# nextpyp/pyp

Measured on AMD Instinct MI355X. Metric: particles/sec projection-matching, 256^2 box, higher is better.
Workload: dtype f32

## Files before the change

pyp_amd/csrc/host_ctx.h:

```cpp
#pragma once

namespace {

thread_local std::string g_err;
int fail(int code, const std::string &msg) { g_err = "ERROR: " + msg; return code; }

#define HIPCHK(call)                                                                          \
    do {                                                                                      \
        hipError_t e_ = (call);                                                               \
        if (e_ != hipSuccess) {                                                               \
            g_err = std::string("ERROR: HIP: ") + hipGetErrorString(e_) + " at " #call;        \
            return -5;                                                                        \
        }                                                                                     \
    } while (0)
#define HIPCHKP(call)                                                                         \
    do {                                                                                      \
        hipError_t e_ = (call);                                                               \
        if (e_ != hipSuccess) {                                                               \
            g_err = std::string("ERROR: HIP: ") + hipGetErrorString(e_) + " at " #call;        \
            return nullptr;                                                                   \
        }                                                                                     \
    } while (0)

struct Ctx {
// ... 112 lines not shown
        if (n <= cap) return 0;
        if (p) (void)hipFree(p);
        p = nullptr; cap = 0;
        HIPCHK(hipMalloc(&p, n * sizeof(T)));
        cap = n;
        return 0;
    }
    void release() { if (p) (void)hipFree(p); p = nullptr; cap = 0; }
};

template <typename T>
struct DevTmp {
    T *p = nullptr;
    DevTmp() = default;
    DevTmp(const DevTmp &) = delete;
    DevTmp &operator=(const DevTmp &) = delete;
    ~DevTmp() { if (p) (void)hipFree(p); }
    hipError_t alloc(size_t n) { return hipMalloc(&p, n * sizeof(T)); }
};


}

struct ppm_ref {
    hipStream_t stream = nullptr, copy = nullptr;
    int N = 0, B = 0, CX = 0, CY = 0, NBX = 0, NBY = 0, pad = 1; unsigned LB = 0;
    float2 *cube = nullptr;
    DevBuf<double> rows_in, rows_out, dir_theta, dir_phi;
    DevBuf<float> images, wring, cw, C2, nP, nI, cc, mats, ddef;
    DevBuf<float2> c_Il, c_band; DevBuf<float> c_cw, c_img, c_wring; DevBuf<double> c_rows, c_N, c_p, c_tl, c_delta, c_s0, c_g0, c_out;
    DevBuf<int> c_eval, c_rp, c_rt, c_slot, c_uoff, c_active; DevBuf<LState> c_states; DevBuf<double> c_mean, c_tmean, c_acc, c_dtrial, c_fpm, c_delta_t;
    DevBuf<float2> s_f, s_g, s_F; DevBuf<float> s_vols;
    struct { bool valid = false; float key[5] = { 0, 0, 0, 0, 0 }; int S = 0; std::vector<int> shell_off; DevBuf<uint32_t> samples, pos; DevBuf<float> bandw; DevBuf<float2> Fw; bool fw_valid = false; float wkey[4] = { 0, 0, 0, 0 }; } s_plan;
    DevBuf<float2> band, Il, Wp, bank, twN;
    DevBuf<float2> spill;
    DevBuf<float4> rowtw;
    DevBuf<int> sh;
    DevBuf<uint32_t> samples;
    DevBuf<Hit> hits, hits_t;
    DevBuf<int> tile_c;
    DevBuf<Hit> hits_s; DevBuf<int> sec_k;
    DevBuf<LState> states, states2;
    DevBuf<float4> bank4; DevBuf<float> part, gtw;
    std::string grid_key, bank_key, bank4_key; int gtw_ns = 0, gtw_rsx = -1;
    long last_counts[4] = { 0, 0, 0, 0 };
    int last_sections = 0;
    std::string note;
};

struct ppm_accum {
    hipStream_t stream = nullptr, copy = nullptr;
    int N = 0; float pixel = 1.f;
    float *acc = nullptr; bool external = false;
    std::vector<double> symops; int nsym = 1;
    float *d_sym = nullptr;
    unsigned long long *d_counts = nullptr;
    unsigned *d_max = nullptr;
    long counts[2] = { 0, 0 };
    DevBuf<double> rows; DevBuf<float> images, dose; DevBuf<float2> band, spill; DevBuf<PartIns> pp; DevBuf<CullEnt> cull; DevBuf<BrickItem> items;
    DevBuf<float2> s_f, s_g; DevBuf<float> s_vols;
    std::vector<float> brick_load; float load_r = -1.f; int n_items = 0, items_cap = -1;
};

static CubeView cube_view(const ppm_ref *ref) {
    CubeView cv;
// ... 4 lines not shown
static bool local_tables_wanted(int tabR) {
    return !(getenv("PPM_LOCAL_TABLES") && atoi(getenv("PPM_LOCAL_TABLES")) == 0) && cube_tab_bytes(tabR) <= 16 * 1024;
}
static bool tables_fit_lds(size_t ring_bytes, int tabR) { return ring_bytes + cube_tab_bytes(tabR) + 2048 <= (size_t)64 * 1024; }

struct ChunkStager {
    const float *src; float *buf; bool on_device; int n_img, chunk; size_t nn;
    int prime() const {
        if (on_device) return 0;
        HIPCHK(hipMemcpyAsync(buf, src, (size_t)std::min(chunk, n_img) * nn * sizeof(float), hipMemcpyHostToDevice, cur_copy()));
        HIPCHK(hipStreamSynchronize(cur_copy()));
        return 0;
    }
    const float *chunk_ptr(int c0, int ci) const { return on_device ? src + (size_t)c0 * nn : buf + (size_t)(ci & 1) * chunk * nn; }
    int prefetch_next(int c0, int ci) const {
        if (on_device || c0 + chunk >= n_img) return 0;
        const int n_next = std::min(chunk, n_img - (c0 + chunk));
        HIPCHK(hipMemcpyAsync(buf + (size_t)((ci + 1) & 1) * chunk * nn, src + (size_t)(c0 + chunk) * nn, (size_t)n_next * nn * sizeof(float), hipMemcpyHostToDevice, cur_copy()));
        return 0;
    }
    int sync() const {
        HIPCHK(hipStreamSynchronize(cur_stream()));
        HIPCHK(hipStreamSynchronize(cur_copy()));
        return 0;
    }
};

static __global__ void k_noop() {}

extern "C" {

const char *ppm_last_error(void) { return g_err.c_str(); }
const char *ppm_version(void) { return "pypmatch 0.1 (gfx950)"; }
const char *ppm_build_id(void) { return "pypmatch " __DATE__ " " __TIME__; }
int ppm_device_mem_info(size_t *free_bytes, size_t *total_bytes) {
    if (!g.inited) return fail(-1, "ppm_init has not been called");
    (void)hipSetDevice(g.device);
    size_t f = 0, t = 0;
    HIPCHK(hipMemGetInfo(&f, &t));
    if (free_bytes) *free_bytes = f;
    if (total_bytes) *total_bytes = t;
    return 0;
}

int ppm_init(int device) {
    static std::mutex init_mu;
// ... 149 lines not shown
```

pyp_amd/csrc/host_refine.h:

```cpp
#pragma once

static int launch_prep(DevBuf<float2> &spill , const float *d_images, const double *d_rows, int n_img, const Geom &gm, double Rm_px, float fall_px,
                       int normalize, int invert, int do_mask, int whiten, float2 *band, float *wring,
                       const uint32_t *samples, int S_pad, float2 *Il, float *cw, float2 *Wp, float *C2, float *nI,
                       unsigned *band_max = nullptr ,
                       const float *focus_px = nullptr ) {
    if (int rc = ensure_plan(gm.N)) return rc;
    PrepP P;
    P.images = d_images; P.rows = d_rows; P.plan = g.plans[gm.N].plan;
    P.N = gm.N; P.B = gm.B; P.W = gm.W; P.H = gm.H;
    P.r_hi2 = (float)(gm.r_hi * gm.r_hi); P.Rm = (float)Rm_px; P.wfall = fall_px; P.a = (float)gm.a;
    P.Rm2_bg = (float)std::min(std::floor(Rm_px * Rm_px), 16777216.0);
    P.normalize = normalize; P.invert = invert; P.do_mask = do_mask; P.whiten = whiten;
    for (int k = 0; k < 4; k++) P.focus[k] = focus_px ? focus_px[k] : 0.f;
    P.band_max = band_max;
    P.band = band; P.wring = wring; P.samples = samples; P.S_pad = S_pad; P.Il = Il; P.cw = cw;
    P.Wp = Wp; P.C2 = C2; P.nI = nI; P.Bs = gm.Bs; P.Hs = gm.Hs;
    P.r_s2 = (float)(gm.r_s * gm.r_s); P.r_lo2 = (float)(gm.r_lo * gm.r_lo);
    const PrepPlan pl = prep_plan(gm.N, gm.B, gm.W);
    if (pl.err) return fail(-12, pl.err);
    P.L = pl.L; P.nc = pl.nc; P.nchunks = pl.nchunks; P.TS = pl.TS; P.WS = pl.WS;
    P.spill = nullptr;
    if (!pl.scratch_free) {
        if (int rc = spill.ensure((size_t)n_img * gm.N * gm.W)) return rc;
// ... 121 lines not shown
    DP.rlo2 = (float)(gm.r_lo * gm.r_lo); DP.rmax2 = (float)(gm.r_hi * gm.r_hi); DP.ring_signed = (float)std::min(gm.ring_signed, 1e30); DP.a = (float)gm.a;
    DP.rows = rows; DP.states = states; DP.ddef = ddef; DP.nt = nt; DP.step = step; DP.all_scores = all_scores; DP.rcls2 = rcls2;
    DP.tchunk = std::max(1, std::min(2 * nt + 1, (int)(60000 / (16 * (size_t)nrings))));
    ProfScope ps(PPM_K_LOCAL);
    hipLaunchKernelGGL(k_defocus, dim3(n), dim3(256), ring_lds_bytes(4, DP.tchunk, nrings), cur_stream(), DP);
}

namespace {
struct RefineRun {
    ppm_ref *ref = nullptr; const ppm_refine_cfg *cfg = nullptr;
    Geom gm; SampleList sl; CubeView cv;
    int S_pad = 0, nrings = 0, CH = 0;
    int K = 0, Tb = 0, Tc = 0;
    double Rm_px = 0; float fall_px = 0;
    bool focus_on = false, sep_search = false; float focus_px[4] = { 0, 0, 0, 0 };
    GfftPlan gpl; bool use_fft = false;
    int Rtx = 0, Rty = 0, Rwin = 0, HsP = 0, nslices = 0; std::vector<int> cxs, cys;
    std::vector<GridSection> secs; std::vector<int> kpre; int sec_dirs = 0;
    LocalP LP; bool local_tab = false;
    double bf = 3.0; bool any_ang = false, any_sh = false;
    int ndef = 0;
    int per_iter = 0; bool cls_on = false;
    double sample_evals = 0;

    int ntiles() const { return (int)(cxs.size() * cys.size()); }
    int nsec() const { return (int)secs.size(); }
    size_t bank_slice() const { return (size_t)HsP * 64; }
    size_t bank4_slice() const { return use_fft ? (size_t)gpl.L * gpl.L : 0; }
    size_t HS() const { return (size_t)gm.Hs * 64; }
    int prefix_of(double rband) const { int rg = (int)std::ceil(rband); if (rg > gm.B + 1) rg = gm.B + 1; return sl.ring_off[rg]; }
};
constexpr int kTileR = 6;
constexpr int kFinalThreads = 256;
}

static void refine_notes(ppm_ref *ref, const ppm_refine_cfg *cfg, const Geom &gm) {
    ref->note.clear();
    if (gm.r_s_asked > gm.r_s) {
        char b[256];
        std::snprintf(b, sizeof(b), "NOTE: global search band lowered from %.1f to %.1f Fourier pixels (%.2f A instead of %.2f A): the grid-search "
                      "kernel covers 64 pixels; the top hits are refined up to the high-resolution limit as asked", gm.r_s_asked, gm.r_s,
                      gm.N * gm.a / gm.r_s, gm.N * gm.a / gm.r_s_asked);
        ref->note = b;
    }
    if (cfg->global_search && gm.range_capped) {
        char b[320];
        std::snprintf(b, sizeof(b), "%sNOTE: shift window of the grid search: +-%.0f x +-%.0f pixels (%d x %d search-grid steps of %.1f pixels, the most the "
                      "search grid of %d points holds; asked: %.0f pixels); the refinement of the hits is not limited to it", ref->note.empty() ? "" : "\n",
                      gm.RSx * gm.step, gm.RSy * gm.step, gm.RSx, gm.RSy, gm.step, gm.Ns, gm.range_asked_px);
        ref->note += b;
    }
}

static size_t workspace_budget() { return g.total_mem / 4; }
static size_t bank_budget() {
    size_t b = g.total_mem / 4;
// ... 49 lines not shown
    HIPCHK(hipMemcpyAsync(ref->samples.p, r.sl.packed.data(), r.S_pad * sizeof(uint32_t), hipMemcpyHostToDevice, cur_stream()));

    r.use_fft = false;
    if (cfg->global_search && gfft_plan(gm, r.gpl)) {
        const char *gp = getenv("PPM_GLOBAL_PATH");
        const bool force_fft = gp && !strcmp(gp, "fft"), force_tiles = gp && !strcmp(gp, "tiles");
        r.use_fft = force_fft || (!force_tiles && std::max(gm.RSx, gm.RSy) > kTileR);
    }
    r.Rtx = std::min(gm.RSx, kTileR); r.Rty = std::min(gm.RSy, kTileR);
    auto tile_centres = [](int RS, int Rt) {
        const int T = (2 * RS + 1 + 2 * Rt) / (2 * Rt + 1);
        std::vector<int> c(T, 0);
        for (int i = 0; i < T && T > 1; i++) c[i] = -RS + Rt + (int)(((long)i * 2 * (RS - Rt)) / (T - 1));
        return c;
    };
    r.cxs = tile_centres(gm.RSx, r.Rtx); r.cys = tile_centres(gm.RSy, r.Rty);
    r.Rwin = std::max(r.Rtx, r.Rty);
    r.HsP = ((2 * (gm.Bs + 1) + 2 * global_unroll(r.Rwin) - 1) / (2 * global_unroll(r.Rwin))) * (2 * global_unroll(r.Rwin));
    r.nslices = gm.n_dir * gm.npsi_store;
    if (cfg->global_search) if (int rc = plan_grid_sections(r)) return rc;
    const size_t NN = (size_t)gm.N * gm.N, HW = (size_t)gm.H * gm.W;
    size_t per = NN * 4 + HW * 8 + (size_t)r.S_pad * 12 + 2 * PPM_NCOL * 8 + (gm.B + 2) * 4;
    if (cfg->global_search) per += r.HS() * 12 + (size_t)r.nslices * 4 + (size_t)gm.n_orient * 8 + (size_t)r.K * (sizeof(Hit) + sizeof(LState)) + sizeof(LState);
    size_t fit = ((size_t)4 << 30) / per;
    if (fit < 64) {
        const size_t ws = workspace_budget(), per_all = per + (r.use_fft ? (size_t)gm.n_orient * 8 : 0);
        fit = std::min<size_t>(64, ws / per_all);
        if (fit < 1) {
            char b[320];
            std::snprintf(b, sizeof(b), "angular step of %.3g degrees: the grid search keeps %.1f GB of tables per particle for its %d orientations, "
                          "the workspace holds %.1f GB; use a coarser angular step", gm.dstep, per_all / 1073741824.0, gm.n_orient, ws / 1073741824.0);
            return fail(-22, b);
        }
    }
    int CH = (int)std::min<size_t>((size_t)n_img, fit);
    CH = std::min(CH, 8192);
    if (CH >= 2048) CH &= ~1023;
    if (const char *e = std::getenv("PPM_CHUNK")) { int v = std::atoi(e); if (v > 0) CH = std::min(CH, v); }
    r.CH = CH;
    return 0;
}

static int ensure_chunk_buffers(RefineRun &r, bool images_on_device) {
    ppm_ref *ref = r.ref; const Geom &gm = r.gm; const int CH = r.CH;
    const size_t NN = (size_t)gm.N * gm.N, HW = (size_t)gm.H * gm.W;
    if (int rc = ref->rows_in.ensure((size_t)CH * PPM_NCOL)) return rc;
    if (int rc = ref->rows_out.ensure((size_t)CH * PPM_NCOL)) return rc;
    if (!images_on_device) if (int rc = ref->images.ensure((size_t)2 * CH * NN)) return rc;
    if (int rc = ref->band.ensure((size_t)CH * HW)) return rc;
    if (int rc = ref->wring.ensure((size_t)CH * (gm.B + 2))) return rc;
    if (int rc = ref->Il.ensure((size_t)CH * r.S_pad)) return rc;
    if (int rc = ref->cw.ensure((size_t)CH * r.S_pad)) return rc;
    if (int rc = ref->states2.ensure(CH)) return rc;
    return 0;
}

static int ensure_bank(RefineRun &r, const GridSection &sec) {
    ppm_ref *ref = r.ref; const Geom &gm = r.gm;
    const std::string key = ref->grid_key + "/d" + std::to_string(sec.d0) + "+" + std::to_string(sec.nd);
    if (ref->bank_key == key) return 0;
    const int nsl = sec.nd * gm.npsi_store;
    BankP BP; BP.cv = r.cv; BP.mats = ref->mats.p + (size_t)sec.d0 * gm.npsi_store * 6; BP.bank = ref->bank.p; BP.nslices = nsl; BP.Bs = gm.Bs; BP.Hs = r.HsP;
    BP.r_s2 = (float)(gm.r_s * gm.r_s);
    {
        ProfScope ps(PPM_K_BANK);
        size_t tot = (size_t)nsl * r.bank_slice();
        hipLaunchKernelGGL(k_bank, dim3((unsigned)((tot + 255) / 256)), dim3(256), 0, cur_stream(), BP);
    }
    HIPCHK(hipGetLastError());
    ref->bank_key = key;
    return 0;
}

static int ensure_bank4(RefineRun &r, const GridSection &sec) {
    ppm_ref *ref = r.ref; const Geom &gm = r.gm; const int L = r.gpl.L;
    const std::string key = ref->grid_key + "/d" + std::to_string(sec.d0) + "+" + std::to_string(sec.nd) + "/L" + std::to_string(L);
    if (ref->bank4_key == key) return 0;
    const int nsl = sec.nd * gm.npsi_store;
    Bank4P BP; BP.cv = r.cv; BP.mats = ref->mats.p + (size_t)sec.d0 * gm.npsi_store * 6; BP.bank4 = ref->bank4.p; BP.nslices = nsl; BP.Bs = gm.Bs; BP.L = L; BP.r_s2 = (float)(gm.r_s * gm.r_s);
    ProfScope ps(PPM_K_BANK);
    const size_t tot = (size_t)nsl * r.bank4_slice();
    hipLaunchKernelGGL(k_bank4, dim3((unsigned)((tot + 255) / 256)), dim3(256), 0, cur_stream(), BP);
    HIPCHK(hipGetLastError());
    ref->bank4_key = key;
    return 0;
}

static int ensure_search_tables(RefineRun &r) {
    ppm_ref *ref = r.ref; const Geom &gm = r.gm; const int CH = r.CH, K = r.K, nslices = r.nslices, HsP = r.HsP;
    const size_t HS = r.HS(), HSP = (size_t)HsP * 64;
    if (int rc = ref->Wp.ensure((size_t)CH * HS)) return rc;
    if (int rc = ref->C2.ensure((size_t)CH * HS)) return rc;
    if (int rc = ref->nP.ensure((size_t)CH * nslices)) return rc;
    if (int rc = ref->nI.ensure(CH)) return rc;
    if (int rc = ref->cc.ensure((size_t)CH * gm.n_orient)) return rc;
    if (int rc = ref->sh.ensure((size_t)CH * gm.n_orient)) return rc;
    if (int rc = ref->hits.ensure((size_t)CH * K)) return rc;
    if (int rc = ref->states.ensure((size_t)CH * K)) return rc;
    {
        const size_t cap = ref->bank.cap;
        if (int rc = ref->bank.ensure((size_t)r.sec_dirs * gm.npsi_store * HSP)) return rc;
        if (ref->bank.cap != cap) ref->bank_key.clear();
    }
    if (r.nsec() > 1) {
        if (int rc = ref->hits_s.ensure((size_t)CH * r.kpre.back())) return rc;
        if (int rc = ref->sec_k.ensure(r.kpre.size())) return rc;
        HIPCHK(hipMemcpyAsync(ref->sec_k.p, r.kpre.data(), r.kpre.size() * sizeof(int), hipMemcpyHostToDevice, cur_stream()));
    }
    char key[160];
    std::snprintf(key, sizeof(key), "%d/%.6f/%.6f/%d/%d/%d/%.3f/%.3f", gm.N, gm.r_s, gm.dstep, gm.Ns, gm.npsi_store, HsP, gm.phi_max, gm.theta_max);
    if (ref->grid_key == key) return 0;
    ref->bank_key.clear(); ref->bank4_key.clear();
    std::vector<float> mats((size_t)nslices * 6);
    std::vector<double> dth(gm.n_dir), dph(gm.n_dir);
    for (int d = 0; d < gm.n_dir; d++) {
        grid_direction(gm, d, dth[d], dph[d]);
        for (int k = 0; k < gm.npsi_store; k++) {
            double M[9]; euler_matrix(k * gm.dpsi, dth[d], dph[d], M);
            float *m = &mats[((size_t)d * gm.npsi_store + k) * 6];
            m[0] = (float)M[0]; m[1] = (float)M[1]; m[2] = (float)M[3]; m[3] = (float)M[4]; m[4] = (float)M[6]; m[5] = (float)M[7];
        }
// ... 41 lines not shown
                for (int j = 1; j <= 3; j++) put(&tw[(size_t)fr::bfly_entry(L, M, k) * 8 + (j - 1) * 2], 2.0 * kPi * j * k / M);
        for (int t = 0; t < L; t++) put(&tw[(size_t)nb * 8 + (size_t)t * 2], 2.0 * kPi * t / gm.Ns);
        for (int pp = 0; pp < L; pp++)
            for (int h = 0; h < 2; h++) {
                const int j = 2 * fr::freq_at(L, pp) + h, sx = j < L ? j : j - gm.Ns;
                tw[(size_t)fr::tw_table_floats(L) + 2 * pp + h] = std::abs(sx) <= gm.RSx ? 0.f : -3.0e38f;
            }
        if (int rc = ref->gtw.ensure(tw.size())) return rc;
        HIPCHK(hipMemcpyAsync(ref->gtw.p, tw.data(), tw.size() * sizeof(float), hipMemcpyHostToDevice, cur_stream()));
        HIPCHK(hipStreamSynchronize(cur_stream()));
        ref->gtw_ns = gm.Ns; ref->gtw_rsx = gm.RSx;
    }
    return 0;
}

static int local_setup(RefineRun &r) {
    ppm_ref *ref = r.ref; const ppm_refine_cfg *cfg = r.cfg; const Geom &gm = r.gm; LocalP &LP = r.LP;
    r.bf = cfg->band_factor == 0 ? 3.0 : cfg->band_factor;
    r.any_ang = cfg->refine_psi || cfg->refine_theta || cfg->refine_phi; r.any_sh = cfg->refine_x || cfg->refine_y;
    r.sample_evals = 0;
    r.ndef = 0;
    if (cfg->refine_defocus && cfg->defocus_step > 0 && cfg->defocus_range >= cfg->defocus_step)
        r.ndef = std::min((int)std::floor(cfg->defocus_range / cfg->defocus_step + 1e-6), PPM_MAX_DEFOCUS_STEPS);
    LP.cv = r.cv; LP.samples = ref->samples.p; LP.Il = ref->Il.p; LP.cw = ref->cw.p; LP.S_pad = r.S_pad; LP.nrings = r.nrings; LP.N = gm.N;
    LP.tabR = cube_tab_radius(gm.B, r.cv.scale);
    r.local_tab = local_tables_wanted(LP.tabR);
    LP.rlo2 = (float)(gm.r_lo * gm.r_lo); LP.ring_signed = (float)std::min(gm.ring_signed, 1e30);
    LP.en[0] = cfg->refine_psi; LP.en[1] = cfg->refine_theta; LP.en[2] = cfg->refine_phi; LP.en[3] = cfg->refine_x; LP.en[4] = cfg->refine_y;
    LP.use_priors = 0;
    for (int i = 0; i < 5; i++) { LP.pmean[i] = 0; LP.pw[i] = 0; }
    if (cfg->use_priors) {
        const double ns = kPi * (gm.r_hi * gm.r_hi - gm.r_lo * gm.r_lo);
        for (int i = 0; i < 5; i++) {
            double var = cfg->prior_var[i], mean = cfg->prior_mean[i];
            if (i >= 3) { mean /= gm.a; var /= gm.a * gm.a; }
            LP.pmean[i] = mean;
            if (LP.en[i] && var > 0 && ns > 0) { LP.pw[i] = 1.0 / (2.0 * var * ns); LP.use_priors = 1; }
        }
    }
    const int nfree = (cfg->refine_psi != 0) + (cfg->refine_theta != 0) + (cfg->refine_phi != 0) + (cfg->refine_x != 0) + (cfg->refine_y != 0);
    r.per_iter = nfree ? 2 * nfree + 2 : 0;
    if (r.Tb + r.Tc > kMaxIters) return fail(-22, "too many compass iterations requested");
    LP.rmax2_final = (float)(gm.r_hi * gm.r_hi); LP.S_final = r.S_pad;
    r.cls_on = gm.r_cls < gm.r_hi;
    LP.rmax2_class = (float)(gm.r_cls * gm.r_cls); LP.S_class = (r.cls_on && r.ndef == 0) ? r.prefix_of(gm.r_cls) : 0;
    return 0;
}
// ... 43 lines not shown
    } else if (ntiles == 1) {
        if (int rc = launch_global(GP, nb, gm.half != 0, r.Rwin)) return rc;
    } else {
        if (int rc = ref->hits_t.ensure((size_t)ntiles * nb * K)) return rc;
        if (int rc = ref->tile_c.ensure((size_t)2 * ntiles)) return rc;
        std::vector<int> tc(2 * ntiles);
        for (int ty = 0, t = 0; ty < (int)r.cys.size(); ty++) for (int tx = 0; tx < (int)r.cxs.size(); tx++, t++) { tc[t] = r.cxs[tx]; tc[ntiles + t] = r.cys[ty]; }
        HIPCHK(hipMemcpyAsync(ref->tile_c.p, tc.data(), tc.size() * sizeof(int), hipMemcpyHostToDevice, cur_stream()));
        int px = 0, py = 0;
        const size_t tot = (size_t)nb * r.HS();
        for (int t = 0; t < ntiles; t++) {
            const int dcx = tc[t] - px, dcy = tc[ntiles + t] - py;
            if (dcx || dcy) hipLaunchKernelGGL(k_wp_ramp, dim3((unsigned)((tot + 255) / 256)), dim3(256), 0, cur_stream(), ref->Wp.p, tot, gm.Bs, gm.Ns, dcx, dcy, ref->twN.p);
            px = tc[t]; py = tc[ntiles + t];
            GP.hits = ref->hits_t.p + (size_t)t * nb * K;
            if (int rc = launch_global(GP, nb, gm.half != 0, r.Rwin)) return rc;
        }
        hipLaunchKernelGGL(k_merge_hits, dim3((nb + 127) / 128), dim3(128), 0, cur_stream(), ref->hits_t.p, hits, nb, K, ntiles, ref->tile_c.p, ref->tile_c.p + ntiles);
        HIPCHK(hipStreamSynchronize(cur_stream()));
    }
    return 0;
}

static int global_stage(RefineRun &r, int nb) {
    ppm_ref *ref = r.ref; const ppm_refine_cfg *cfg = r.cfg; const Geom &gm = r.gm; LocalP &LP = r.LP;
    const int K = r.K, Tb = r.Tb, Tc = r.Tc;
    if (r.nsec() == 1) {
        if (int rc = search_section(r, nb, r.secs[0], ref->hits.p, K)) return rc;
    } else {
        for (int s = 0; s < r.nsec(); s++)
            if (int rc = search_section(r, nb, r.secs[s], ref->hits_s.p + (size_t)r.kpre[s] * nb, r.kpre[s + 1] - r.kpre[s])) return rc;
        ProfScope ps(PPM_K_TOPK);
        hipLaunchKernelGGL(k_merge_sections, dim3(nb), dim3(64), 0, cur_stream(), ref->hits_s.p, ref->hits.p, nb, K, r.nsec(), ref->sec_k.p);
        HIPCHK(hipGetLastError());
    }
    {
        ProfScope ps(PPM_K_TOPK);
        hipLaunchKernelGGL(k_states_from_hits, dim3((nb * K + 255) / 256), dim3(256), 0, cur_stream(), ref->hits.p, ref->states.p, nb, K,
                           ref->dir_theta.p, ref->dir_phi.p, gm.n_psi, gm.dpsi, gm.step, 0.5 * gm.dstep, gm.step);
    }
    r.sample_evals = 0;
    if (Tb > 0) {
        LP.states = ref->states.p; LP.T = Tb; LP.final_rescore = 0;
        LP.nr = std::min(r.nrings, (int)std::ceil(gm.r_s) + 1);
        fill_schedule(r, 0.5 * gm.dstep, gm.step, Tb, gm.r_s, (double)K);
        ProfScope ps(PPM_K_LOCAL);
        launch_local(r, (unsigned)(nb * K), LP.S_it[0] <= 1024 ? 64 : 128);
    }
    {
        ProfScope ps(PPM_K_TOPK);
        hipLaunchKernelGGL(k_select_best, dim3((nb + 255) / 256), dim3(256), 0, cur_stream(), ref->states.p, ref->states2.p, nb, K);
    }
    LP.states = ref->states2.p; LP.T = cfg->local_refine ? Tc : 0; LP.final_rescore = 1; LP.nr = r.nrings;
    fill_schedule(r, 0.5 * gm.dstep / (double)(1 << Tb), gm.step / (double)(1 << Tb), LP.T, gm.r_hi, 1.0);
    r.sample_evals += std::floor(kPi * gm.r_hi * gm.r_hi / 2);
    ProfScope ps(PPM_K_LOCAL);
    launch_local(r, (unsigned)nb, kFinalThreads);
    return 0;
}

static void rows_stage(RefineRun &r, int nb) {
    ppm_ref *ref = r.ref; const ppm_refine_cfg *cfg = r.cfg; const Geom &gm = r.gm; LocalP &LP = r.LP;
    double ha0 = cfg->local_angle_step > 0 ? cfg->local_angle_step : 2.5, hs0 = cfg->local_shift_step > 0 ? cfg->local_shift_step : 2.0;
    hipLaunchKernelGGL(k_states_from_rows, dim3((nb + 255) / 256), dim3(256), 0, cur_stream(), ref->rows_in.p, ref->states2.p, nb, gm.a, ha0, hs0);
    r.sample_evals = 0;
    LP.states = ref->states2.p; LP.T = cfg->local_refine ? r.Tb + r.Tc : 0; LP.final_rescore = 1; LP.nr = r.nrings;
    fill_schedule(r, ha0, hs0, LP.T, gm.r_hi, 1.0);
    r.sample_evals += std::floor(kPi * gm.r_hi * gm.r_hi / 2);
    ProfScope ps(PPM_K_LOCAL);
    launch_local(r, (unsigned)nb, kFinalThreads);
}

static int finish_chunk(RefineRun &r, int nb) {
    ppm_ref *ref = r.ref; const Geom &gm = r.gm;
    const float *d_ddef = nullptr;
    if (r.ndef > 0) {
        if (int rc = ref->ddef.ensure(r.CH)) return rc;
        launch_defocus(r.cv, gm, ref->samples.p, r.S_pad, ref->Il.p, ref->wring.p, ref->rows_in.p, ref->states2.p, nb, r.ndef, r.cfg->defocus_step,
                       ref->ddef.p, nullptr, r.cls_on ? (float)(gm.r_cls * gm.r_cls) : 0.f);
        d_ddef = ref->ddef.p;
    }
    hipLaunchKernelGGL(k_rows_out, dim3((nb + 255) / 256), dim3(256), 0, cur_stream(), ref->states2.p, ref->rows_in.p, ref->rows_out.p, nb, gm.a, gm.r_cls, gm.r_lo, d_ddef);
    HIPCHK(hipGetLastError());
    return 0;
}

static void refine_counts(RefineRun &r) {
    const ppm_refine_cfg *cfg = r.cfg; const Geom &gm = r.gm;
    long nl;
    if (cfg->global_search) nl = (long)r.K * r.Tb * r.per_iter + (cfg->local_refine ? (long)r.Tc * r.per_iter : 0) + 1;
    else nl = 1 + (cfg->local_refine ? (long)(r.Tb + r.Tc) * r.per_iter : 0);
    r.ref->last_counts[0] = cfg->global_search ? gm.n_orient : 0;
    nl += 2L * r.ndef + (r.cls_on ? 1 : 0);
    if (r.cls_on) r.sample_evals += std::floor(kPi * gm.r_cls * gm.r_cls / 2);
    r.sample_evals += 2.0 * r.ndef * std::floor(kPi * gm.r_hi * gm.r_hi / 2);
    r.ref->last_counts[1] = nl;
    r.ref->last_counts[2] = (long)std::floor(kPi * gm.r_s * gm.r_s / 2);
    r.ref->last_counts[3] = (long)r.sample_evals;
}

extern "C" {

ppm_ref_t *ppm_reference_create_weighted(const float *vol, int n, float max_band_px, int pad, const float *ring_weight, int n_weight) {
    if (!g.inited) { fail(-1, "ppm_init has not been called"); return nullptr; }
    if (!vol || !box_ok(n) || !(max_band_px > 0)) { fail(-22, "reference box must be even, 32..512, with prime factors 2, 3, 5, 7, and the band positive"); return nullptr; }
    if ((pad != 1 && pad != 2 && pad != 4) || n * pad > 512) { fail(-22, "padding factor must be 1, 2 or 4 with padded box <= 512"); return nullptr; }
    if (max_band_px > n / 2) max_band_px = (float)(n / 2);
    const int np = n * pad;
    int B = (int)std::ceil((double)max_band_px * pad) - 1;
    if (B > np / 2 - 1) B = np / 2 - 1;
    size_t n3 = (size_t)n * n * n, np3 = (size_t)np * np * np;
    std::unique_ptr<ppm_ref, void (*)(ppm_ref_t *)> guard(new ppm_ref(), ppm_reference_destroy);
    ppm_ref *r = guard.get();
    HIPCHKP(hipStreamCreateWithFlags(&r->stream, hipStreamNonBlocking));
    HIPCHKP(hipStreamCreateWithFlags(&r->copy, hipStreamNonBlocking));
    StreamScope ss_(r->stream, r->copy);
    DevTmp<float> t_vol, t_w; DevTmp<float2> t_f;
    HIPCHKP(t_vol.alloc(n3));
    HIPCHKP(t_f.alloc(np3));
    float *d_vol = t_vol.p; float2 *d_f = t_f.p;
    HIPCHKP(hipMemcpy(d_vol, vol, n3 * sizeof(float), hipMemcpyHostToDevice));
    if (pad > 1) HIPCHKP(hipMemsetAsync(d_f, 0, np3 * sizeof(float2), cur_stream()));
    float *d_w = nullptr;
    if (ring_weight && n_weight > 0) {
        HIPCHKP(t_w.alloc((size_t)n_weight));
        d_w = t_w.p;
        HIPCHKP(hipMemcpyAsync(d_w, ring_weight, (size_t)n_weight * sizeof(float), hipMemcpyHostToDevice, cur_stream()));
    }
    r->N = n; r->pad = pad; r->B = B; r->CX = B + 2; r->CY = 2 * B + 3;
    size_t cube_n = (size_t)r->CX * r->CY * r->CY;
    r->NBX = (r->CX + 3) / 4; r->NBY = (r->CY + 1) / 2;
    const size_t copy_n = (size_t)r->NBX * r->NBY * r->NBY * 16;
    if (2 * copy_n * sizeof(float2) >= ((size_t)1 << 32)) {
    fail(-22, "reference cube too large"); return nullptr; }
    r->LB = (unsigned)copy_n;
    if (hipMalloc(&r->cube, 2 * copy_n * sizeof(float2)) != hipSuccess) { r->cube = nullptr; fail(-12, "out of device memory for the reference cube"); return nullptr; }
    HIPCHKP(hipMemsetAsync(r->cube, 0, 2 * copy_n * sizeof(float2), cur_stream()));
    {
        ProfScope ps(PPM_K_BANK);
        hipLaunchKernelGGL(k_ref_load, dim3((unsigned)((n3 + 255) / 256)), dim3(256), 0, cur_stream(), d_vol, d_f, n, np);
        if (fft3d(d_f, np, false)) return nullptr;
        hipLaunchKernelGGL(k_ref_crop, dim3((unsigned)((cube_n + 255) / 256)), dim3(256), 0, cur_stream(), d_f, r->cube, np, n, B, r->CX, r->CY, r->NBX, r->NBY, r->LB, d_w, n_weight);
    }
    if (hipStreamSynchronize(cur_stream()) != hipSuccess || hipGetLastError() != hipSuccess) { fail(-5, "reference preparation failed on the device"); return nullptr; }
    return guard.release();
}

ppm_ref_t *ppm_reference_create_padded(const float *vol, int n, float max_band_px, int pad) { return ppm_reference_create_weighted(vol, n, max_band_px, pad, nullptr, 0); }
ppm_ref_t *ppm_reference_create(const float *vol, int n, float max_band_px) { return ppm_reference_create_weighted(vol, n, max_band_px, 1, nullptr, 0); }

void ppm_reference_destroy(ppm_ref_t *r) {
    if (!r) return;
    if (r->cube) (void)hipFree(r->cube);
    r->rows_in.release(); r->rows_out.release(); r->dir_theta.release(); r->dir_phi.release();
    r->images.release(); r->wring.release(); r->cw.release(); r->C2.release(); r->nP.release(); r->nI.release();
    r->s_f.release(); r->s_g.release(); r->s_F.release(); r->s_vols.release(); r->s_plan.samples.release(); r->s_plan.pos.release(); r->s_plan.bandw.release(); r->s_plan.Fw.release();
    r->c_Il.release(); r->c_band.release(); r->c_cw.release(); r->c_img.release(); r->c_wring.release(); r->c_rows.release(); r->c_N.release(); r->c_p.release(); r->c_tl.release();
    r->c_delta.release(); r->c_s0.release(); r->c_g0.release(); r->c_out.release(); r->c_eval.release(); r->c_rp.release(); r->c_rt.release(); r->c_slot.release(); r->c_states.release(); r->c_uoff.release(); r->c_mean.release(); r->c_active.release(); r->c_tmean.release(); r->c_acc.release(); r->c_dtrial.release(); r->c_fpm.release(); r->c_delta_t.release(); r->cc.release(); r->mats.release(); r->ddef.release();
    r->band.release(); r->spill.release(); r->Il.release(); r->Wp.release(); r->bank.release(); r->twN.release(); r->rowtw.release(); r->sh.release(); r->samples.release();
    r->hits.release(); r->states.release(); r->states2.release();
    r->hits_t.release(); r->tile_c.release(); r->hits_s.release(); r->sec_k.release(); r->bank4.release(); r->part.release(); r->gtw.release();
    if (r->stream) (void)hipStreamDestroy(r->stream);
    if (r->copy) (void)hipStreamDestroy(r->copy);
    delete r;
}

int ppm_match_projections(ppm_ref_t *ref, const ppm_refine_cfg *cfg, const double *rows, int n_rows, float *out) {
    if (!g.inited) return fail(-1, "ppm_init has not been called");
    if (!ref || !cfg || !rows || !out) return fail(-22, "null argument");
    StreamScope ss_(ref->stream, ref->copy);
    if (n_rows <= 0) return 0;
    ppm_refine_cfg c2 = *cfg; c2.global_search = 0;
    Geom gm; std::string err;
    if (!geom_init(gm, c2, err)) return fail(-22, err);
    if (gm.N != ref->N) return fail(-22, "particle box differs from the reference box");
    if (gm.B > (ref->B + 1) / ref->pad - 1) return fail(-22, "high-resolution limit exceeds the band the reference was prepared for");
    const size_t NN = (size_t)gm.N * gm.N;
    const int CH = (int)std::min<size_t>((size_t)n_rows, std::max<size_t>(1, ((size_t)1 << 30) / (NN * 12)));
    DevTmp<float2> d_f; DevTmp<float> d_o; DevTmp<MatchRow> d_rows;
    HIPCHK(d_f.alloc(NN * CH)); HIPCHK(d_o.alloc(NN * CH)); HIPCHK(d_rows.alloc(CH));
    MatchP MP;
    MP.cv = cube_view(ref);
    MP.rows = d_rows.p; MP.f = d_f.p; MP.N = gm.N; MP.B = gm.B; MP.r_hi2 = (float)(gm.r_hi * gm.r_hi);
    std::vector<MatchRow> hr(CH);
    const float scale = (cfg->invert ? -1.f : 1.f) / (float)gm.N;
    for (int c0 = 0; c0 < n_rows; c0 += CH) {
// ... 24 lines not shown
    if (!ref || !cfg || !images || !rows_in || !rows_out) return fail(-22, "null argument");
    StreamScope ss_(ref->stream, ref->copy);
    if (n_img <= 0) return 0;
    ref->last_sections = 0;
    RefineRun r; r.ref = ref; r.cfg = cfg;
    const Geom &gm = r.gm; std::string err;
    if (!geom_init(r.gm, *cfg, err)) return fail(-22, err);
    if (gm.N != ref->N) return fail(-22, "particle box differs from the reference box");
    refine_notes(ref, cfg, gm);
    if (gm.B > (ref->B + 1) / ref->pad - 1) return fail(-22, "high-resolution limit exceeds the band the reference was prepared for");
    if (cfg->global_search && gm.Bs + 1 > 64)
        return fail(-22, "global search band wider than 64 Fourier pixels is not supported; lower the 'resolution limit for search'");
    if (int rc = refine_plan(r, n_img)) return rc;
    if (int rc = ensure_chunk_buffers(r, images_on_device != 0)) return rc;
    r.cv = cube_view(ref);
    if (cfg->global_search) {
        if (int rc = ensure_search_tables(r)) return rc;
        if (int rc = ensure_bank(r, r.secs[0])) return rc;
        if (r.use_fft) { if (int rc = ensure_gfft_tables(r)) return rc; if (int rc = ensure_bank4(r, r.secs[0])) return rc; }
    }
    HIPCHK(hipStreamSynchronize(cur_stream()));
    if (int rc = local_setup(r)) return rc;

    const int CH = r.CH;
    const size_t NN = (size_t)gm.N * gm.N;
    const ChunkStager stage{ (const float *)images, ref->images.p, images_on_device != 0, n_img, CH, NN };
    if (int rc = stage.prime()) return rc;
    for (int c0 = 0, ci = 0; c0 < n_img; c0 += CH, ci++) {
        const int nb = std::min(CH, n_img - c0);
        HIPCHK(hipMemcpyAsync(ref->rows_in.p, rows_in + (size_t)c0 * PPM_NCOL, (size_t)nb * PPM_NCOL * sizeof(double), hipMemcpyHostToDevice, cur_stream()));
        const float *d_img = stage.chunk_ptr(c0, ci);
        if (int rc = launch_prep(ref->spill, d_img, ref->rows_in.p, nb, gm, r.Rm_px, r.fall_px, cfg->normalize, cfg->invert, 1, 1, ref->band.p, ref->wring.p,
                                 ref->samples.p, r.S_pad, ref->Il.p, ref->cw.p,
                                 (cfg->global_search && !r.sep_search) ? ref->Wp.p : nullptr, ref->C2.p, ref->nI.p, nullptr, r.focus_on ? r.focus_px : nullptr)) return rc;
        if (r.sep_search)
            if (int rc = launch_prep(ref->spill, d_img, ref->rows_in.p, nb, gm, cfg->search_mask_radius / gm.a, r.fall_px, cfg->normalize, cfg->invert, 1, 1,
                                     ref->band.p, nullptr, nullptr, 0, nullptr, nullptr, ref->Wp.p, ref->C2.p, ref->nI.p)) return rc;
        if (cfg->global_search) { if (int rc = global_stage(r, nb)) return rc; }
        else rows_stage(r, nb);
        if (int rc = finish_chunk(r, nb)) return rc;
        if (int rc = stage.prefetch_next(c0, ci)) return rc;
        HIPCHK(hipMemcpyAsync(rows_out + (size_t)c0 * PPM_NCOL, ref->rows_out.p, (size_t)nb * PPM_NCOL * sizeof(double), hipMemcpyDeviceToHost, cur_stream()));
        if (int rc = stage.sync()) return rc;
    }
    refine_counts(r);
    return 0;
}


const char *ppm_refine_note(ppm_ref_t *ref) { return ref ? ref->note.c_str() : ""; }

int ppm_refine_last_sections(ppm_ref_t *ref) { return ref ? ref->last_sections : 0; }

int ppm_refine_last_counts(ppm_ref_t *ref, long *n_global, long *n_local, long *samples_global, long *samples_local) {
    if (!ref) return fail(-22, "null reference");
    if (n_global) *n_global = ref->last_counts[0];
    if (n_local) *n_local = ref->last_counts[1];
    if (samples_global) *samples_global = ref->last_counts[2];
    if (samples_local) *samples_local = ref->last_counts[3];
    return 0;
}

}
```

Measured before the change: 79040.

## Double-buffer refine chunk state and pipeline search with local refinement

Per-chunk buffers (rows, Il, cw, wring, hits, states) move into two ChunkSets with events, so the search stage of chunk i+1 can be issued before the local refinement of chunk i. Image uploads are scheduled two chunks ahead, gated on events, and the per-chunk full host synchronisation becomes a wait on the previous chunk's event only. Running the local stage on a separate stream needs the PPM_REFINE_OVERLAP env var; by default both stages share the main stream but are still queued without per-chunk host stalls. The doubled per-particle workspace can shrink the chunk size.

```diff
diff --git a/pyp_amd/csrc/host_ctx.h b/pyp_amd/csrc/host_ctx.h
--- a/pyp_amd/csrc/host_ctx.h
+++ b/pyp_amd/csrc/host_ctx.h
@@ -158,25 +158,39 @@
 
 }
 
+struct ChunkSet {
+    DevBuf<double> rows_in, rows_out;
+    DevBuf<float2> Il; DevBuf<float> cw, wring, ddef;
+    DevBuf<Hit> hits; DevBuf<LState> states, states2;
+    hipEvent_t hits_ready = nullptr, local_done = nullptr;
+    void release() {
+        rows_in.release(); rows_out.release(); Il.release(); cw.release(); wring.release(); ddef.release(); hits.release(); states.release(); states2.release();
+        if (hits_ready) (void)hipEventDestroy(hits_ready);
+        if (local_done) (void)hipEventDestroy(local_done);
+        hits_ready = local_done = nullptr;
+    }
+};
+
 struct ppm_ref {
     hipStream_t stream = nullptr, copy = nullptr;
+    hipStream_t local = nullptr;
+    ChunkSet cs[2];
     int N = 0, B = 0, CX = 0, CY = 0, NBX = 0, NBY = 0, pad = 1; unsigned LB = 0;
     float2 *cube = nullptr;
-    DevBuf<double> rows_in, rows_out, dir_theta, dir_phi;
-    DevBuf<float> images, wring, cw, C2, nP, nI, cc, mats, ddef;
+    DevBuf<double> dir_theta, dir_phi;
+    DevBuf<float> images, C2, nP, nI, cc, mats;
     DevBuf<float2> c_Il, c_band; DevBuf<float> c_cw, c_img, c_wring; DevBuf<double> c_rows, c_N, c_p, c_tl, c_delta, c_s0, c_g0, c_out;
     DevBuf<int> c_eval, c_rp, c_rt, c_slot, c_uoff, c_active; DevBuf<LState> c_states; DevBuf<double> c_mean, c_tmean, c_acc, c_dtrial, c_fpm, c_delta_t;
     DevBuf<float2> s_f, s_g, s_F; DevBuf<float> s_vols;
     struct { bool valid = false; float key[5] = { 0, 0, 0, 0, 0 }; int S = 0; std::vector<int> shell_off; DevBuf<uint32_t> samples, pos; DevBuf<float> bandw; DevBuf<float2> Fw; bool fw_valid = false; float wkey[4] = { 0, 0, 0, 0 }; } s_plan;
-    DevBuf<float2> band, Il, Wp, bank, twN;
+    DevBuf<float2> band, Wp, bank, twN;
     DevBuf<float2> spill;
     DevBuf<float4> rowtw;
     DevBuf<int> sh;
     DevBuf<uint32_t> samples;
-    DevBuf<Hit> hits, hits_t;
+    DevBuf<Hit> hits_t;
     DevBuf<int> tile_c;
     DevBuf<Hit> hits_s; DevBuf<int> sec_k;
-    DevBuf<LState> states, states2;
     DevBuf<float4> bank4; DevBuf<float> part, gtw;
     std::string grid_key, bank_key, bank4_key; int gtw_ns = 0, gtw_rsx = -1;
     long last_counts[4] = { 0, 0, 0, 0 };
@@ -227,6 +241,17 @@
     int sync() const {
         HIPCHK(hipStreamSynchronize(cur_stream()));
         HIPCHK(hipStreamSynchronize(cur_copy()));
+        return 0;
+    }
+    int upload(int ci, hipEvent_t half_free) const {
+        const size_t c0 = (size_t)ci * chunk;
+        if (on_device || c0 >= (size_t)n_img) return 0;
+        if (half_free) HIPCHK(hipStreamWaitEvent(cur_copy(), half_free, 0));
+        HIPCHK(hipMemcpyAsync(buf + (size_t)(ci & 1) * chunk * nn, src + c0 * nn, std::min((size_t)chunk, (size_t)n_img - c0) * nn * sizeof(float), hipMemcpyHostToDevice, cur_copy()));
+        return 0;
+    }
+    int wait_uploads() const {
+        if (!on_device) HIPCHK(hipStreamSynchronize(cur_copy()));
         return 0;
     }
 };
diff --git a/pyp_amd/csrc/host_refine.h b/pyp_amd/csrc/host_refine.h
--- a/pyp_amd/csrc/host_refine.h
+++ b/pyp_amd/csrc/host_refine.h
@@ -167,6 +167,7 @@
     int ndef = 0;
     int per_iter = 0; bool cls_on = false;
     double sample_evals = 0;
+    bool overlap = false;
 
     int ntiles() const { return (int)(cxs.size() * cys.size()); }
     int nsec() const { return (int)secs.size(); }
@@ -177,6 +178,8 @@
 };
 constexpr int kTileR = 6;
 constexpr int kFinalThreads = 256;
+
+struct ChunkJob { int c0 = 0, nb = 0, ci = 0; ChunkSet *set = nullptr; };
 }
 
 static void refine_notes(ppm_ref *ref, const ppm_refine_cfg *cfg, const Geom &gm) {
@@ -272,6 +275,7 @@
     const size_t NN = (size_t)gm.N * gm.N, HW = (size_t)gm.H * gm.W;
     size_t per = NN * 4 + HW * 8 + (size_t)r.S_pad * 12 + 2 * PPM_NCOL * 8 + (gm.B + 2) * 4;
     if (cfg->global_search) per += r.HS() * 12 + (size_t)r.nslices * 4 + (size_t)gm.n_orient * 8 + (size_t)r.K * (sizeof(Hit) + sizeof(LState)) + sizeof(LState);
+    per += (size_t)r.S_pad * 12 + 2 * PPM_NCOL * 8 + (gm.B + 2) * 4 + sizeof(LState) + (cfg->global_search ? (size_t)r.K * (sizeof(Hit) + sizeof(LState)) : 0);
     size_t fit = ((size_t)4 << 30) / per;
     if (fit < 64) {
         const size_t ws = workspace_budget(), per_all = per + (r.use_fft ? (size_t)gm.n_orient * 8 : 0);
@@ -288,20 +292,27 @@
     if (CH >= 2048) CH &= ~1023;
     if (const char *e = std::getenv("PPM_CHUNK")) { int v = std::atoi(e); if (v > 0) CH = std::min(CH, v); }
     r.CH = CH;
+    if (getenv("PPM_TRACE")) fprintf(stderr, "ppm_refine_batch: chunks of %d particles (%zu workspace bytes per particle)\n", CH, per);
     return 0;
 }
 
 static int ensure_chunk_buffers(RefineRun &r, bool images_on_device) {
     ppm_ref *ref = r.ref; const Geom &gm = r.gm; const int CH = r.CH;
     const size_t NN = (size_t)gm.N * gm.N, HW = (size_t)gm.H * gm.W;
-    if (int rc = ref->rows_in.ensure((size_t)CH * PPM_NCOL)) return rc;
-    if (int rc = ref->rows_out.ensure((size_t)CH * PPM_NCOL)) return rc;
     if (!images_on_device) if (int rc = ref->images.ensure((size_t)2 * CH * NN)) return rc;
     if (int rc = ref->band.ensure((size_t)CH * HW)) return rc;
-    if (int rc = ref->wring.ensure((size_t)CH * (gm.B + 2))) return rc;
-    if (int rc = ref->Il.ensure((size_t)CH * r.S_pad)) return rc;
-    if (int rc = ref->cw.ensure((size_t)CH * r.S_pad)) return rc;
-    if (int rc = ref->states2.ensure(CH)) return rc;
+    for (ChunkSet &cs : ref->cs) {
+        if (int rc = cs.rows_in.ensure((size_t)CH * PPM_NCOL)) return rc;
+        if (int rc = cs.rows_out.ensure((size_t)CH * PPM_NCOL)) return rc;
+        if (int rc = cs.wring.ensure((size_t)CH * (gm.B + 2))) return rc;
+        if (int rc = cs.Il.ensure((size_t)CH * r.S_pad)) return rc;
+        if (int rc = cs.cw.ensure((size_t)CH * r.S_pad)) return rc;
+        if (int rc = cs.states2.ensure(CH)) return rc;
+        if (r.cfg->global_search) {
+            if (int rc = cs.hits.ensure((size_t)CH * r.K)) return rc;
+            if (int rc = cs.states.ensure((size_t)CH * r.K)) return rc;
+        }
+    }
     return 0;
 }
 
@@ -337,7 +348,7 @@
 }
 
 static int ensure_search_tables(RefineRun &r) {
-    ppm_ref *ref = r.ref; const Geom &gm = r.gm; const int CH = r.CH, K = r.K, nslices = r.nslices, HsP = r.HsP;
+    ppm_ref *ref = r.ref; const Geom &gm = r.gm; const int CH = r.CH, nslices = r.nslices, HsP = r.HsP;
     const size_t HS = r.HS(), HSP = (size_t)HsP * 64;
     if (int rc = ref->Wp.ensure((size_t)CH * HS)) return rc;
     if (int rc = ref->C2.ensure((size_t)CH * HS)) return rc;
@@ -345,8 +356,6 @@
     if (int rc = ref->nI.ensure(CH)) return rc;
     if (int rc = ref->cc.ensure((size_t)CH * gm.n_orient)) return rc;
     if (int rc = ref->sh.ensure((size_t)CH * gm.n_orient)) return rc;
-    if (int rc = ref->hits.ensure((size_t)CH * K)) return rc;
-    if (int rc = ref->states.ensure((size_t)CH * K)) return rc;
     {
         const size_t cap = ref->bank.cap;
         if (int rc = ref->bank.ensure((size_t)r.sec_dirs * gm.npsi_store * HSP)) return rc;
@@ -434,7 +443,7 @@
     r.ndef = 0;
     if (cfg->refine_defocus && cfg->defocus_step > 0 && cfg->defocus_range >= cfg->defocus_step)
         r.ndef = std::min((int)std::floor(cfg->defocus_range / cfg->defocus_step + 1e-6), PPM_MAX_DEFOCUS_STEPS);
-    LP.cv = r.cv; LP.samples = ref->samples.p; LP.Il = ref->Il.p; LP.cw = ref->cw.p; LP.S_pad = r.S_pad; LP.nrings = r.nrings; LP.N = gm.N;
+    LP.cv = r.cv; LP.samples = ref->samples.p; LP.S_pad = r.S_pad; LP.nrings = r.nrings; LP.N = gm.N;
     LP.tabR = cube_tab_radius(gm.B, r.cv.scale);
     r.local_tab = local_tables_wanted(LP.tabR);
     LP.rlo2 = (float)(gm.r_lo * gm.r_lo); LP.ring_signed = (float)std::min(gm.ring_signed, 1e30);
@@ -524,26 +533,29 @@
     return 0;
 }
 
-static int global_stage(RefineRun &r, int nb) {
+static int search_hits(RefineRun &r, const ChunkJob &j) {
+    ppm_ref *ref = r.ref;
+    const int nb = j.nb, K = r.K;
+    if (r.nsec() == 1) return search_section(r, nb, r.secs[0], j.set->hits.p, K);
+    for (int s = 0; s < r.nsec(); s++)
+        if (int rc = search_section(r, nb, r.secs[s], ref->hits_s.p + (size_t)r.kpre[s] * nb, r.kpre[s + 1] - r.kpre[s])) return rc;
+    ProfScope ps(PPM_K_TOPK);
+    hipLaunchKernelGGL(k_merge_sections, dim3(nb), dim3(64), 0, cur_stream(), ref->hits_s.p, j.set->hits.p, nb, K, r.nsec(), ref->sec_k.p);
+    HIPCHK(hipGetLastError());
+    return 0;
+}
+
+static void refine_hits(RefineRun &r, const ChunkJob &j) {
     ppm_ref *ref = r.ref; const ppm_refine_cfg *cfg = r.cfg; const Geom &gm = r.gm; LocalP &LP = r.LP;
-    const int K = r.K, Tb = r.Tb, Tc = r.Tc;
-    if (r.nsec() == 1) {
-        if (int rc = search_section(r, nb, r.secs[0], ref->hits.p, K)) return rc;
-    } else {
-        for (int s = 0; s < r.nsec(); s++)
-            if (int rc = search_section(r, nb, r.secs[s], ref->hits_s.p + (size_t)r.kpre[s] * nb, r.kpre[s + 1] - r.kpre[s])) return rc;
-        ProfScope ps(PPM_K_TOPK);
-        hipLaunchKernelGGL(k_merge_sections, dim3(nb), dim3(64), 0, cur_stream(), ref->hits_s.p, ref->hits.p, nb, K, r.nsec(), ref->sec_k.p);
-        HIPCHK(hipGetLastError());
-    }
+    const int nb = j.nb, K = r.K, Tb = r.Tb, Tc = r.Tc;
     {
         ProfScope ps(PPM_K_TOPK);
-        hipLaunchKernelGGL(k_states_from_hits, dim3((nb * K + 255) / 256), dim3(256), 0, cur_stream(), ref->hits.p, ref->states.p, nb, K,
+        hipLaunchKernelGGL(k_states_from_hits, dim3((nb * K + 255) / 256), dim3(256), 0, cur_stream(), j.set->hits.p, j.set->states.p, nb, K,
                            ref->dir_theta.p, ref->dir_phi.p, gm.n_psi, gm.dpsi, gm.step, 0.5 * gm.dstep, gm.step);
     }
     r.sample_evals = 0;
     if (Tb > 0) {
-        LP.states = ref->states.p; LP.T = Tb; LP.final_rescore = 0;
+        LP.states = j.set->states.p; LP.T = Tb; LP.final_rescore = 0;
         LP.nr = std::min(r.nrings, (int)std::ceil(gm.r_s) + 1);
         fill_schedule(r, 0.5 * gm.dstep, gm.step, Tb, gm.r_s, (double)K);
         ProfScope ps(PPM_K_LOCAL);
@@ -551,40 +563,76 @@
     }
     {
         ProfScope ps(PPM_K_TOPK);
-        hipLaunchKernelGGL(k_select_best, dim3((nb + 255) / 256), dim3(256), 0, cur_stream(), ref->states.p, ref->states2.p, nb, K);
-    }
-    LP.states = ref->states2.p; LP.T = cfg->local_refine ? Tc : 0; LP.final_rescore = 1; LP.nr = r.nrings;
+        hipLaunchKernelGGL(k_select_best, dim3((nb + 255) / 256), dim3(256), 0, cur_stream(), j.set->states.p, j.set->states2.p, nb, K);
+    }
+    LP.states = j.set->states2.p; LP.T = cfg->local_refine ? Tc : 0; LP.final_rescore = 1; LP.nr = r.nrings;
     fill_schedule(r, 0.5 * gm.dstep / (double)(1 << Tb), gm.step / (double)(1 << Tb), LP.T, gm.r_hi, 1.0);
     r.sample_evals += std::floor(kPi * gm.r_hi * gm.r_hi / 2);
     ProfScope ps(PPM_K_LOCAL);
     launch_local(r, (unsigned)nb, kFinalThreads);
-    return 0;
-}
-
-static void rows_stage(RefineRun &r, int nb) {
-    ppm_ref *ref = r.ref; const ppm_refine_cfg *cfg = r.cfg; const Geom &gm = r.gm; LocalP &LP = r.LP;
+}
+
+static void refine_rows(RefineRun &r, const ChunkJob &j) {
+    const ppm_refine_cfg *cfg = r.cfg; const Geom &gm = r.gm; LocalP &LP = r.LP;
+    const int nb = j.nb;
     double ha0 = cfg->local_angle_step > 0 ? cfg->local_angle_step : 2.5, hs0 = cfg->local_shift_step > 0 ? cfg->local_shift_step : 2.0;
-    hipLaunchKernelGGL(k_states_from_rows, dim3((nb + 255) / 256), dim3(256), 0, cur_stream(), ref->rows_in.p, ref->states2.p, nb, gm.a, ha0, hs0);
+    hipLaunchKernelGGL(k_states_from_rows, dim3((nb + 255) / 256), dim3(256), 0, cur_stream(), j.set->rows_in.p, j.set->states2.p, nb, gm.a, ha0, hs0);
     r.sample_evals = 0;
-    LP.states = ref->states2.p; LP.T = cfg->local_refine ? r.Tb + r.Tc : 0; LP.final_rescore = 1; LP.nr = r.nrings;
+    LP.states = j.set->states2.p; LP.T = cfg->local_refine ? r.Tb + r.Tc : 0; LP.final_rescore = 1; LP.nr = r.nrings;
     fill_schedule(r, ha0, hs0, LP.T, gm.r_hi, 1.0);
     r.sample_evals += std::floor(kPi * gm.r_hi * gm.r_hi / 2);
     ProfScope ps(PPM_K_LOCAL);
     launch_local(r, (unsigned)nb, kFinalThreads);
 }
 
-static int finish_chunk(RefineRun &r, int nb) {
-    ppm_ref *ref = r.ref; const Geom &gm = r.gm;
+static int finish_chunk(RefineRun &r, const ChunkJob &j) {
+    ppm_ref *ref = r.ref; const Geom &gm = r.gm; ChunkSet &cs = *j.set;
+    const int nb = j.nb;
     const float *d_ddef = nullptr;
     if (r.ndef > 0) {
-        if (int rc = ref->ddef.ensure(r.CH)) return rc;
-        launch_defocus(r.cv, gm, ref->samples.p, r.S_pad, ref->Il.p, ref->wring.p, ref->rows_in.p, ref->states2.p, nb, r.ndef, r.cfg->defocus_step,
-                       ref->ddef.p, nullptr, r.cls_on ? (float)(gm.r_cls * gm.r_cls) : 0.f);
-        d_ddef = ref->ddef.p;
-    }
-    hipLaunchKernelGGL(k_rows_out, dim3((nb + 255) / 256), dim3(256), 0, cur_stream(), ref->states2.p, ref->rows_in.p, ref->rows_out.p, nb, gm.a, gm.r_cls, gm.r_lo, d_ddef);
+        if (int rc = cs.ddef.ensure(r.CH)) return rc;
+        launch_defocus(r.cv, gm, ref->samples.p, r.S_pad, cs.Il.p, cs.wring.p, cs.rows_in.p, cs.states2.p, nb, r.ndef, r.cfg->defocus_step,
+                       cs.ddef.p, nullptr, r.cls_on ? (float)(gm.r_cls * gm.r_cls) : 0.f);
+        d_ddef = cs.ddef.p;
+    }
+    hipLaunchKernelGGL(k_rows_out, dim3((nb + 255) / 256), dim3(256), 0, cur_stream(), cs.states2.p, cs.rows_in.p, cs.rows_out.p, nb, gm.a, gm.r_cls, gm.r_lo, d_ddef);
     HIPCHK(hipGetLastError());
     return 0;
+}
+
+static int search_stage(RefineRun &r, const ChunkStager &stage, const ChunkJob &j, const double *rows_in) {
+    ppm_ref *ref = r.ref; const ppm_refine_cfg *cfg = r.cfg; const Geom &gm = r.gm; ChunkSet &cs = *j.set;
+    HIPCHK(hipStreamWaitEvent(cur_stream(), cs.local_done, 0));
+    HIPCHK(hipMemcpyAsync(cs.rows_in.p, rows_in + (size_t)j.c0 * PPM_NCOL, (size_t)j.nb * PPM_NCOL * sizeof(double), hipMemcpyHostToDevice, cur_stream()));
+    if (int rc = stage.wait_uploads()) return rc;
+    const float *d_img = stage.chunk_ptr(j.c0, j.ci);
+    if (int rc = launch_prep(ref->spill, d_img, cs.rows_in.p, j.nb, gm, r.Rm_px, r.fall_px, cfg->normalize, cfg->invert, 1, 1, ref->band.p, cs.wring.p,
+                             ref->samples.p, r.S_pad, cs.Il.p, cs.cw.p,
+                             (cfg->global_search && !r.sep_search) ? ref->Wp.p : nullptr, ref->C2.p, ref->nI.p, nullptr, r.focus_on ? r.focus_px : nullptr)) return rc;
+    if (r.sep_search)
+        if (int rc = launch_prep(ref->spill, d_img, cs.rows_in.p, j.nb, gm, cfg->search_mask_radius / gm.a, r.fall_px, cfg->normalize, cfg->invert, 1, 1,
+                                 ref->band.p, nullptr, nullptr, 0, nullptr, nullptr, ref->Wp.p, ref->C2.p, ref->nI.p)) return rc;
+    if (cfg->global_search) if (int rc = search_hits(r, j)) return rc;
+    HIPCHK(hipEventRecord(cs.hits_ready, cur_stream()));
+    return 0;
+}
+
+static int local_stage(RefineRun &r, const ChunkJob &j, double *rows_out) {
+    ppm_ref *ref = r.ref; ChunkSet &cs = *j.set;
+    StreamScope on_local(r.overlap ? ref->local : ref->stream, ref->copy);
+    HIPCHK(hipStreamWaitEvent(cur_stream(), cs.hits_ready, 0));
+    r.LP.Il = cs.Il.p; r.LP.cw = cs.cw.p;
+    if (r.cfg->global_search) refine_hits(r, j);
+    else refine_rows(r, j);
+    if (int rc = finish_chunk(r, j)) return rc;
+    HIPCHK(hipMemcpyAsync(rows_out + (size_t)j.c0 * PPM_NCOL, cs.rows_out.p, (size_t)j.nb * PPM_NCOL * sizeof(double), hipMemcpyDeviceToHost, cur_stream()));
+    HIPCHK(hipEventRecord(cs.local_done, cur_stream()));
+    return 0;
+}
+
+static bool refine_overlap_wanted() {
+    const char *e = getenv("PPM_REFINE_OVERLAP");
+    return e && atoi(e) != 0;
 }
 
 static void refine_counts(RefineRun &r) {
@@ -616,6 +664,11 @@
     ppm_ref *r = guard.get();
     HIPCHKP(hipStreamCreateWithFlags(&r->stream, hipStreamNonBlocking));
     HIPCHKP(hipStreamCreateWithFlags(&r->copy, hipStreamNonBlocking));
+    HIPCHKP(hipStreamCreateWithFlags(&r->local, hipStreamNonBlocking));
+    for (ChunkSet &cs : r->cs) {
+        HIPCHKP(hipEventCreateWithFlags(&cs.hits_ready, hipEventDisableTiming));
+        HIPCHKP(hipEventCreateWithFlags(&cs.local_done, hipEventDisableTiming));
+    }
     StreamScope ss_(r->stream, r->copy);
     DevTmp<float> t_vol, t_w; DevTmp<float2> t_f;
     HIPCHKP(t_vol.alloc(n3));
@@ -654,16 +707,17 @@
 void ppm_reference_destroy(ppm_ref_t *r) {
     if (!r) return;
     if (r->cube) (void)hipFree(r->cube);
-    r->rows_in.release(); r->rows_out.release(); r->dir_theta.release(); r->dir_phi.release();
-    r->images.release(); r->wring.release(); r->cw.release(); r->C2.release(); r->nP.release(); r->nI.release();
+    for (ChunkSet &cs : r->cs) cs.release();
+    r->dir_theta.release(); r->dir_phi.release();
+    r->images.release(); r->C2.release(); r->nP.release(); r->nI.release();
     r->s_f.release(); r->s_g.release(); r->s_F.release(); r->s_vols.release(); r->s_plan.samples.release(); r->s_plan.pos.release(); r->s_plan.bandw.release(); r->s_plan.Fw.release();
     r->c_Il.release(); r->c_band.release(); r->c_cw.release(); r->c_img.release(); r->c_wring.release(); r->c_rows.release(); r->c_N.release(); r->c_p.release(); r->c_tl.release();
-    r->c_delta.release(); r->c_s0.release(); r->c_g0.release(); r->c_out.release(); r->c_eval.release(); r->c_rp.release(); r->c_rt.release(); r->c_slot.release(); r->c_states.release(); r->c_uoff.release(); r->c_mean.release(); r->c_active.release(); r->c_tmean.release(); r->c_acc.release(); r->c_dtrial.release(); r->c_fpm.release(); r->c_delta_t.release(); r->cc.release(); r->mats.release(); r->ddef.release();
-    r->band.release(); r->spill.release(); r->Il.release(); r->Wp.release(); r->bank.release(); r->twN.release(); r->rowtw.release(); r->sh.release(); r->samples.release();
-    r->hits.release(); r->states.release(); r->states2.release();
+    r->c_delta.release(); r->c_s0.release(); r->c_g0.release(); r->c_out.release(); r->c_eval.release(); r->c_rp.release(); r->c_rt.release(); r->c_slot.release(); r->c_states.release(); r->c_uoff.release(); r->c_mean.release(); r->c_active.release(); r->c_tmean.release(); r->c_acc.release(); r->c_dtrial.release(); r->c_fpm.release(); r->c_delta_t.release(); r->cc.release(); r->mats.release();
+    r->band.release(); r->spill.release(); r->Wp.release(); r->bank.release(); r->twN.release(); r->rowtw.release(); r->sh.release(); r->samples.release();
     r->hits_t.release(); r->tile_c.release(); r->hits_s.release(); r->sec_k.release(); r->bank4.release(); r->part.release(); r->gtw.release();
     if (r->stream) (void)hipStreamDestroy(r->stream);
     if (r->copy) (void)hipStreamDestroy(r->copy);
+    if (r->local) (void)hipStreamDestroy(r->local);
     delete r;
 }
 
@@ -734,27 +788,24 @@
     HIPCHK(hipStreamSynchronize(cur_stream()));
     if (int rc = local_setup(r)) return rc;
 
-    const int CH = r.CH;
+    r.overlap = cfg->global_search && refine_overlap_wanted();
+    const int CH = r.CH, nchunks = (n_img + CH - 1) / CH;
     const size_t NN = (size_t)gm.N * gm.N;
     const ChunkStager stage{ (const float *)images, ref->images.p, images_on_device != 0, n_img, CH, NN };
+    auto job = [&](int ci) { ChunkJob j; j.c0 = ci * CH; j.nb = std::min(CH, n_img - j.c0); j.ci = ci; j.set = &ref->cs[ci & 1]; return j; };
+    struct Drain { ppm_ref *ref; ~Drain() { (void)hipStreamSynchronize(ref->stream); (void)hipStreamSynchronize(ref->local); (void)hipStreamSynchronize(ref->copy); } } drain{ ref };
     if (int rc = stage.prime()) return rc;
-    for (int c0 = 0, ci = 0; c0 < n_img; c0 += CH, ci++) {
-        const int nb = std::min(CH, n_img - c0);
-        HIPCHK(hipMemcpyAsync(ref->rows_in.p, rows_in + (size_t)c0 * PPM_NCOL, (size_t)nb * PPM_NCOL * sizeof(double), hipMemcpyHostToDevice, cur_stream()));
-        const float *d_img = stage.chunk_ptr(c0, ci);
-        if (int rc = launch_prep(ref->spill, d_img, ref->rows_in.p, nb, gm, r.Rm_px, r.fall_px, cfg->normalize, cfg->invert, 1, 1, ref->band.p, ref->wring.p,
-                                 ref->samples.p, r.S_pad, ref->Il.p, ref->cw.p,
-                                 (cfg->global_search && !r.sep_search) ? ref->Wp.p : nullptr, ref->C2.p, ref->nI.p, nullptr, r.focus_on ? r.focus_px : nullptr)) return rc;
-        if (r.sep_search)
-            if (int rc = launch_prep(ref->spill, d_img, ref->rows_in.p, nb, gm, cfg->search_mask_radius / gm.a, r.fall_px, cfg->normalize, cfg->invert, 1, 1,
-                                     ref->band.p, nullptr, nullptr, 0, nullptr, nullptr, ref->Wp.p, ref->C2.p, ref->nI.p)) return rc;
-        if (cfg->global_search) { if (int rc = global_stage(r, nb)) return rc; }
-        else rows_stage(r, nb);
-        if (int rc = finish_chunk(r, nb)) return rc;
-        if (int rc = stage.prefetch_next(c0, ci)) return rc;
-        HIPCHK(hipMemcpyAsync(rows_out + (size_t)c0 * PPM_NCOL, ref->rows_out.p, (size_t)nb * PPM_NCOL * sizeof(double), hipMemcpyDeviceToHost, cur_stream()));
-        if (int rc = stage.sync()) return rc;
-    }
+    if (int rc = stage.upload(1, nullptr)) return rc;
+    if (int rc = search_stage(r, stage, job(0), rows_in)) return rc;
+    for (int ci = 0; ci < nchunks; ci++) {
+        if (ci + 1 < nchunks) if (int rc = search_stage(r, stage, job(ci + 1), rows_in)) return rc;
+        if (int rc = local_stage(r, job(ci), rows_out)) return rc;
+        if (int rc = stage.upload(ci + 2, ref->cs[ci & 1].hits_ready)) return rc;
+        if (ci > 0) HIPCHK(hipEventSynchronize(ref->cs[(ci - 1) & 1].local_done));
+    }
+    HIPCHK(hipStreamSynchronize(r.overlap ? ref->local : ref->stream));
+    HIPCHK(hipStreamSynchronize(ref->stream));
+    HIPCHK(hipGetLastError());
     refine_counts(r);
     return 0;
 }
```

New measurement: 78400. No clear change (-0.8%).
